# focegueda1998/CALM-ViT-DTE

Hardware: AMD Instinct MI355X
Metric: training images/sec (224^2, bs=256/GPU) (higher is better)
Workload: dtype f32; 1 GPU; CALM-ViT small224 cls, 224x224x3 synthetic, bs=256/GPU, fp32 matmuls, fwd+loss+bwd+clip+AdamW; batch resident in HBM when the timed region starts (the trainer's H2D copy of the batch is excluded); global_batch=256, parallelism=dp1, world=1, backend=none (single process), hipgraph=False

## Files before the change

calm-vit-dte_amd/_lib.py:

```python
import ctypes as C
import os

HERE = os.path.dirname(os.path.abspath(__file__))
LIB_PATH = os.environ.get("CALM_VIT_LIB") or os.path.join(HERE, "libcalmvit_hip.so")

ACT_NONE, ACT_GELU, ACT_GELU_BWD = 0, 1, 2
F32 = 0
ST_F32, ST_BF16, ST_FP8_E4M3, ST_FP8_E5M2 = 0, 1, 2, 3
E_INVAL, E_LAYOUT, E_UNSUPP = -1, -2, -3
ABI_VERSION = 7

_p = C.c_void_p
_i32 = C.c_int32
_i64 = C.c_int64
_f32 = C.c_float


class GemmArgs(C.Structure):
    _fields_ = [
        ("A", _p), ("B", _p), ("C", _p),
        ("M", _i32), ("N", _i32), ("K", _i32),
        ("batch0", _i32), ("batch1", _i32),
        ("a_rs", _i64), ("a_cs", _i64), ("a_b0", _i64), ("a_b1", _i64),
        ("b_rs", _i64), ("b_cs", _i64), ("b_b0", _i64), ("b_b1", _i64),
# ... 78 lines not shown
    "calm_gemm": (_i32, [C.POINTER(GemmArgs), _p]),
    "calm_gemm_workspace_bytes": (_i64, [C.POINTER(GemmArgs)]),
    "calm_gemm_set_option": (C.c_int, [_i32, _i32]),
    "calm_gemm_describe": (_i32, [C.POINTER(GemmArgs), C.POINTER(GemmPlan)]),
    "calm_reduce_scratch_floats": (_i64, [_i32, _i64, _i32]),
    "calm_layernorm_fwd": (_i32, [_p, _p, _p, _p, _p, _i64, _i32, _f32, _i32, _p]),
    "calm_layernorm_bwd": (_i32, [_p, _p, _p, _p, _p, _p, _p, _p, _i64, _i32, _i32, _p, _p]),
    "calm_cast_chunk_elems": (_i32, []),
    "calm_cast_bf16": (_i32, [_p, _p, _i32, _p]),
    "calm_cast_bf16_one": (_i32, [_p, _p, _i64, _p]),
    "calm_cast_f32_one": (_i32, [_p, _p, _i64, _p]),
    "calm_quantize_fp8": (_i32, [_p, _i32, _i64, _p, _i32, _p, _p]),
    "calm_transpose_u8": (_i32, [_p, _p, _i32, _i32, _p]),
    "calm_rope_fwd": (_i32, [_p, _p, _p, _p, _p, _i32, _i32, _i32, _i32, _i32, _i32, _i32, _i32, _p]),
    "calm_rope_bwd": (_i32, [_p, _p, _p, _p, _p, _p, _i32, _i32, _i32, _i32, _i32, _i32, _i32, _i32, _i32, _p, _p]),
    "calm_softmax_fwd": (_i32, [_p, _i64, _i32, _p]),
    "calm_softmax_bwd": (_i32, [_p, _p, _i64, _i32, _p]),
    "calm_softmax_bwd_heads": (_i32, [_p, _p, _p, _i32, _i32, _i32, _i32, _p]),
    "calm_sum_heads": (_i32, [_p, _p, _i32, _i32, _i64, _p]),
    "calm_attention_fwd_supported": (_i32, [_i32, _i32, _i32, _i32]),
    "calm_attention_fwd": (_i32, [_p] * 15 + [_i32] * 5 + [_p]),
    "calm_attention_bwd_preferred": (_i32, [_i32, _i32, _i32, _i32]),
    "calm_attention_bwd": (_i32, [_p] * 10 + [_i32] * 5 + [_p]),
    "calm_attention_fwd_lse": (_i32, [_p] * 15 + [_i32] * 5 + [_p]),
    "calm_attention_bwd_lse_scratch_bytes": (_i64, [_i32] * 5),
    "calm_attention_bwd_lse": (_i32, [_p] * 7 + [_i64] + [_p] * 4 + [_i32] * 5 + [_p]),
    "calm_attention_infer": (_i32, [_p] * 11 + [_i32] * 5 + [_p]),
    "calm_attention16_supported": (_i32, [_i32, _i32, _i32]),
    "calm_attention16_fwd": (_i32, [_p] * 16 + [_i32] * 4 + [_p]),
    "calm_attention16_bwd": (_i32, [_p] * 13 + [_i32] * 4 + [_p]),
    "calm_attention16_infer": (_i32, [_p] * 11 + [_i32] * 4 + [_p]),
    "calm_latent_fwd": (_i32, [_p, _p, _p, _p, _p, _i64, _i32, _p, _p]),
    "calm_latent_bwd": (_i32, [_p, _p, _p, _p, _p, _p, _i64, _i32, _p]),
    "calm_sn_plan": (_i32, [C.POINTER(SnLayer), _i32, _p, C.POINTER(SnPlanInfo)]),
    "calm_sn_power_iter": (_i32, [_p, C.POINTER(SnPlanInfo), _i32, _f32, _p, _p]),
    "calm_sn_weight_bwd": (_i32, [_p, _p, _p, _p, _p, _p, _p, _p, _i32, _i32, _p, _p]),
    "calm_optim_chunk_elems": (_i32, []),
    "calm_optim_step": (_i32, [_p, _i32, _p, _i32, _p, C.POINTER(OptimHparams), _p, _p, _p, _p, _p]),
    "calm_ema_chunk_elems": (_i32, []),
    "calm_ema_update": (_i32, [_p, _i32, _p, _i32, _f32, _i32, _p, _p, _p, _p]),
    "calm_ema_swap": (_i32, [_p, _i32, _p, _i32, _p]),
    "calm_collate_mix": (_i32, [_p, _p, _p, _i32, _i32, _i32, _i32, _f32, _p, _p, _p, _p]),
    "calm_collate_crop_mix": (_i32, [_p, _i32, _i32, _p, _p, _p, _i32, _i32, _i32, _i32, _i32, _f32, _p, _p, _p, _p]),
    "calm_augment_collate": (_i32, [_p, _i32, _i32, _p, _p, _p, _i32, _i32, _i32, _i32, _i32, _f32, _p, _p, _p, _p]),
    "calm_resize_coeffs": (_i32, [_i32, _i32, _p, _p, _i32]),
    "calm_resize_u8": (_i32, [_p, _i64, _p, _p, _i32, _i32, _i32, _p]),
# ... 51 lines not shown
```

calm-vit-dte_amd/backend.py:

```python
import contextlib
import ctypes as C
import os

import numpy as np
import torch

from . import _lib
from ._lib import ACT_GELU, ACT_GELU_BWD, ACT_NONE

SN_EPS = 1e-12

GEMM_WORKSPACE = os.environ.get("CALM_GEMM_WORKSPACE", "1") != "0"
BF16_STORAGE = os.environ.get("CALM_BF16_STORAGE", "1") != "0"
PRECISIONS = {"fp32": 0, "bf16": 1, "bf16x3": 2, "fp8": 1}
FP8_DTYPES = (torch.float8_e4m3fn, torch.float8_e5m2)
_precision = "fp32"


def set_matmul_precision(name):
    global _precision
    if name not in PRECISIONS:
        raise ValueError(f"unknown matmul precision {name!r}; choose from {sorted(PRECISIONS)}")
    _precision = name

# ... 1 lines not shown
def get_matmul_precision():
    return _precision


ATTENTION_STORAGES = ("probs", "lse")


def _check_attention_storage(name):
    if name not in ATTENTION_STORAGES:
        raise ValueError(f"unknown attention storage {name!r}; choose from {sorted(ATTENTION_STORAGES)}")
    return name


_attention_storage = _check_attention_storage(os.environ.get("CALM_ATTN_STORAGE") or "probs")


def set_attention_storage(name):
    global _attention_storage
    _attention_storage = _check_attention_storage(name)


def get_attention_storage():
    return _attention_storage


_lean_inference = os.environ.get("CALM_LEAN_INFERENCE", "0") not in ("", "0")


def set_lean_inference(on):
    global _lean_inference
    _lean_inference = bool(on)


def get_lean_inference():
    return _lean_inference


def lean_forward():
    return _lean_inference and not torch.is_grad_enabled()


_loss_kernels = os.environ.get("CALM_LOSS_KERNELS", "0") not in ("", "0")


def set_loss_kernels(on):
    global _loss_kernels
# ... 541 lines not shown
    def softmax_bwd_heads(self, p, dp, dm, B, H, Sq, cols):
        _lib.check(self.lib.calm_softmax_bwd_heads(_ptr(p), _ptr(dp), _ptr(dm), B, H, Sq, cols, _stream()),
                   "calm_softmax_bwd_heads")

    def sum_heads(self, dl, dm, B, H, per_head):
        _lib.check(self.lib.calm_sum_heads(_ptr(dl), _ptr(dm), B, H, per_head, _stream()), "calm_sum_heads")

    def attn_fwd_supported(self, Sq, Skv, H, hd):
        return bool(self.lib.calm_attention_fwd_supported(Sq, Skv, H, hd))

    def attn_fwd(self, q, k, v, w1, b1, s1, w2, b2, s2, out, R, hp, hg, Mk, P, B, Sq, Skv, H, hd):
        _lib.check(self.lib.calm_attention_fwd(_ptr(q), _ptr(k), _ptr(v), _ptr(w1), _ptr(b1), _ptr(s1), _ptr(w2),
                                               _ptr(b2), _ptr(s2), _ptr(out), _ptr(R), _ptr(hp), _ptr(hg),
                                               _ptr(Mk), _ptr(P, True), B, Sq, Skv, H, hd, _stream()), "calm_attention_fwd")

    def attn_bwd_preferred(self, Sq, Skv, H, hd):
        return bool(self.lib.calm_attention_bwd_preferred(Sq, Skv, H, hd))

    def attn_bwd(self, q, k, v, dout, P, dS, dq, dk, dv, dM, B, Sq, Skv, H, hd):
        _lib.check(self.lib.calm_attention_bwd(_ptr(q), _ptr(k), _ptr(v), _ptr(dout), _ptr(P), _ptr(dS), _ptr(dq),
                                               _ptr(dk), _ptr(dv), _ptr(dM), B, Sq, Skv, H, hd, _stream()),
                   "calm_attention_bwd")

    def attn_fwd_lse(self, q, k, v, w1, b1, s1, w2, b2, s2, out, R, hp, hg, Mk, lse, B, Sq, Skv, H, hd):
        _lib.check(self.lib.calm_attention_fwd_lse(_ptr(q), _ptr(k), _ptr(v), _ptr(w1), _ptr(b1), _ptr(s1), _ptr(w2),
                                                   _ptr(b2), _ptr(s2), _ptr(out), _ptr(R), _ptr(hp), _ptr(hg),
                                                   _ptr(Mk), _ptr(lse), B, Sq, Skv, H, hd, _stream()),
                   "calm_attention_fwd_lse")

    def attn_bwd_lse_scratch_bytes(self, B, Sq, Skv, H, hd):
        return int(self.lib.calm_attention_bwd_lse_scratch_bytes(B, Sq, Skv, H, hd))

    def attn_bwd_lse(self, q, k, v, dout, Mk, lse, scratch, dq, dk, dv, dM, B, Sq, Skv, H, hd):
        if scratch is None or not scratch.is_cuda or not scratch.is_contiguous():
            raise TypeError("attn_bwd_lse: contiguous CUDA scratch tensor expected")
        _lib.check(self.lib.calm_attention_bwd_lse(_ptr(q), _ptr(k), _ptr(v), _ptr(dout), _ptr(Mk), _ptr(lse),
                                                   scratch.data_ptr(), scratch.numel() * scratch.element_size(),
                                                   _ptr(dq), _ptr(dk), _ptr(dv), _ptr(dM), B, Sq, Skv, H, hd, _stream()),
                   "calm_attention_bwd_lse")

    def attn_infer(self, q, k, v, w1, b1, s1, w2, b2, s2, out, Mk, B, Sq, Skv, H, hd):
        _lib.check(self.lib.calm_attention_infer(_ptr(q), _ptr(k), _ptr(v), _ptr(w1), _ptr(b1), _ptr(s1), _ptr(w2),
                                                 _ptr(b2), _ptr(s2), _ptr(out), _ptr(Mk), B, Sq, Skv, H, hd, _stream()),
                   "calm_attention_infer")

    def attn16_supported(self, S, H, hd):
# ... 164 lines not shown
```

calm-vit-dte_amd/csrc/attention_fused.hip:

```cpp
#include "common.h"

#ifndef ATT_TR_ROWFAST
#define ATT_TR_ROWFAST 1
#endif

namespace {

typedef float f32x4v __attribute__((ext_vector_type(4)));

struct AttnFwdP {
    const float* q; const float* k; const float* v;
    const float* w1; const float* b1; const float* s1;
    const float* w2; const float* b2; const float* s2;
    float* out;
    float* R; float* hp; float* hg; float* Mk; float* P;
    int B, Sq, Skv, H, hd;
    float scale;
    float* lse;
};

constexpr int NV_Q = 1;

template <int NV> struct Regs { f32x4v v[NV]; };

// ... 73 lines not shown
    static constexpr int SKV = 16 * NJ, TQ = 16 * NW;
    static constexpr int LDJ = ld_km(SKV), LDQ = ld_km(TQ);
    static constexpr int LDN1 = 20;
    static constexpr int LDJ2 = SKV + 4;
    static_assert(LDJ % 32 == 16 && LDQ % 32 == 16, "K-major strides: lane groups 16 banks apart");
    static constexpr int Q_OFF = 32 * LDJ, V_OFF = Q_OFF + 32 * LDQ;
    __device__ static float* buf_k(float* smem, int i) { return smem + i * 16 * LDJ; }
    __device__ static float* buf_q(float* smem, int i) { return smem + Q_OFF + i * 16 * LDQ; }
    static constexpr int W2_OFF = 2 * SKV * LDN1, PH2 = W2_OFF + 32 * LDJ2;
    __device__ static float* buf_w1(float* smem, int i) { return smem + i * SKV * LDN1; }
    __device__ static float* buf_w2(float* smem, int i) { return smem + W2_OFF + i * 16 * LDJ2; }
    struct Hd { int DT, hdp, LDV, stripe; };
    __host__ __device__ static constexpr Hd at(int hd) {
        const int DT = (hd + 15) / 16;
        const int hdp = 16 * DT, LDV = hdp + 4;
        return {DT, hdp, LDV, SKV * LDV};
    }
    static constexpr size_t fwd_bytes(int hd) {
        const int ph13 = V_OFF + at(hd).stripe;
        return sizeof(float) * (size_t)(ph13 > PH2 ? ph13 : PH2);
    }
    static constexpr size_t bwd_q_bytes(int hd) { return sizeof(float) * (size_t)(V_OFF + at(hd).stripe); }
    static constexpr size_t bwd_kv_bytes(int hd) { return sizeof(float) * (size_t)at(hd).stripe; }
};

template <int NJ, int NW, bool LEAN>
__global__ __launch_bounds__(64 * NW) void attn_fwd_kernel(const AttnFwdP p) {
    constexpr int NTH = 64 * NW;
    constexpr int NV_K = (NJ + NW - 1) / NW;
    extern __shared__ __attribute__((aligned(16))) float smem[];
    typedef AttGeo<NJ, NW> G;
    constexpr int SKV = G::SKV, LDJ = G::LDJ, LDN1 = G::LDN1, LDJ2 = G::LDJ2;

    const int tid = threadIdx.x, lane = tid & 63, wave = tid >> 6;
    constexpr int TQ = G::TQ, LDQ = G::LDQ;
    const int r16 = lane & 15, g = lane >> 4;
    const int b = blockIdx.y;
    const int q0 = blockIdx.x * TQ;
    const int nq = min(TQ, p.Sq - q0);
    const bool active = 16 * wave < nq;
    const int iq = q0 + 16 * wave + r16;
    const int D = p.H * p.hd;

    const float* qb = p.q + ((long)b * p.Sq + q0) * D;
    const float* kb = p.k + (long)b * p.Skv * D;
    const float* vb = p.v + (long)b * p.Skv * D;
// ... 238 lines not shown
                    for (int r = 0; r < 4; ++r) {
                        accO = MFMA16(vcol[(16 * t + 4 * g + r) * LDV], accS[t][r], accO);
                        accO2 = MFMA16(vcol[(16 * t + 4 * g + r) * LDV + d2], accS[t][r], accO2);
                    }
                if (16 * d + 4 * g < hd) *reinterpret_cast<f32x4v*>(orow + 16 * d + 4 * g) = accO;
                if (d + 1 < DT && 16 * (d + 1) + 4 * g < hd)
                    *reinterpret_cast<f32x4v*>(orow + 16 * (d + 1) + 4 * g) = accO2;
            }
        }
        __syncthreads();
    }
}

struct AttnBwdP {
    const float* q; const float* k; const float* v; const float* dout;
    const float* P;
    float* dS;
    float* dq; float* dk; float* dv;
    float* dM;
    int B, Sq, Skv, H, hd;
    float scale;
    const float* Mk;
    const float* lse;
};

template <int NJ, int NW, bool LSE>
__global__ __launch_bounds__(64 * NW) void attn_bwd_q_kernel(const AttnBwdP p) {
    constexpr int NTH = 64 * NW;
    constexpr int NV_K = (NJ + NW - 1) / NW;
    extern __shared__ __attribute__((aligned(16))) float smem[];
    typedef AttGeo<NJ, NW> G;
    constexpr int SKV = G::SKV, LDJ = G::LDJ, TQ = G::TQ, LDQ = G::LDQ;
    const int tid = threadIdx.x, lane = tid & 63, wave = tid >> 6;
    const int r16 = lane & 15, g = lane >> 4;
    const int b = blockIdx.y;
    const int q0 = blockIdx.x * TQ;
    const int nq = min(TQ, p.Sq - q0);
    const bool active = 16 * wave < nq;
    const int iq = q0 + 16 * wave + r16;
    const int D = p.H * p.hd;
    const int hd = p.hd;
    const auto gh = G::at(hd);
    const int DT = gh.DT, hdp = gh.hdp, LDV = gh.LDV;
    auto bufK = [&](int i) { return G::buf_k(smem, i); };
    auto bufQ = [&](int i) { return G::buf_q(smem, i); };
    float* bufV = smem + G::V_OFF;
// ... 174 lines not shown
                const float* kcol = bufV + 16 * d + r16;
                const int d2 = (d + 1 < DT) ? 16 : 0;
#pragma unroll
                for (int t = 0; t < NJ; ++t)
#pragma unroll
                    for (int r = 0; r < 4; ++r) {
                        accO = MFMA16(kcol[(16 * t + 4 * g + r) * LDV], accD[t][r], accO);
                        accO2 = MFMA16(kcol[(16 * t + 4 * g + r) * LDV + d2], accD[t][r], accO2);
                    }
                if (16 * d + 4 * g < hd) *reinterpret_cast<f32x4v*>(qrow + 16 * d + 4 * g) = accO * p.scale;
                if (d + 1 < DT && 16 * (d + 1) + 4 * g < hd)
                    *reinterpret_cast<f32x4v*>(qrow + 16 * (d + 1) + 4 * g) = accO2 * p.scale;
            }
        }
        __syncthreads();
    }
    if (active) {
        float* mrow = p.dM + ((long)b * p.Sq + iq) * p.Skv;
#pragma unroll
        for (int t = 0; t < NJ; ++t) *reinterpret_cast<f32x4v*>(mrow + 16 * t + 4 * g) = accM[t];
    }
}

template <int NI, int NW>
__global__ __launch_bounds__(64 * NW) void attn_bwd_kv_kernel(const AttnBwdP p) {
    constexpr int NTH = 64 * NW;
    extern __shared__ __attribute__((aligned(16))) float smem[];
    typedef AttGeo<NI, NW> G;
    constexpr int SQ = G::SKV, TK = G::TQ;
    const int tid = threadIdx.x, lane = tid & 63, wave = tid >> 6;
    const int r16 = lane & 15, g = lane >> 4;
    const int b = blockIdx.y;
    const int k0 = blockIdx.x * TK;
    const int nk = min(TK, p.Skv - k0);
    const bool active = 16 * wave < nk;
    const int jk = k0 + 16 * wave + r16;
    const int D = p.H * p.hd;
    const int hd = p.hd;
    const auto gh = G::at(hd);
    const int DT = gh.DT, hdp = gh.hdp, LDV = gh.LDV;
    float* bufV = smem;
    const int v_per_row = hdp >> 2, v_total = SQ * v_per_row;
    const float* qb = p.q + (long)b * p.Sq * D;
    const float* dob = p.dout + (long)b * p.Sq * D;

    constexpr int SB = 4;
    auto stage = [&](const float* src) {
#pragma unroll 1
        for (int f0 = tid; f0 < v_total; f0 += SB * NTH) {
            f32x4v val[SB];
#pragma unroll
            for (int u = 0; u < SB; ++u) {
                const int f = f0 + u * NTH;
                const int row = f / v_per_row, cq = f - row * v_per_row;
                val[u] = (f32x4v){0.f, 0.f, 0.f, 0.f};
                if (f < v_total && 4 * cq < hd) val[u] = *reinterpret_cast<const f32x4v*>(src + (long)row * D + 4 * cq);
            }
#pragma unroll
            for (int u = 0; u < SB; ++u) {
                const int f = f0 + u * NTH;
                const int row = f / v_per_row, cq = f - row * v_per_row;
                if (f < v_total) *reinterpret_cast<f32x4v*>(bufV + row * LDV + 4 * cq) = val[u];
            }
        }
    };
    auto contract = [&](const f32x4v (&X)[NI], float* out_row, float scale) {
#pragma unroll 1
        for (int d = 0; d < DT; d += 2) {
            f32x4v accO = {0.f, 0.f, 0.f, 0.f}, accO2 = {0.f, 0.f, 0.f, 0.f};
            const float* col = bufV + 16 * d + r16;
            const int d2 = (d + 1 < DT) ? 16 : 0;
#pragma unroll
            for (int t = 0; t < NI; ++t)
#pragma unroll
                for (int r = 0; r < 4; ++r) {
                    accO = MFMA16(col[(16 * t + 4 * g + r) * LDV], X[t][r], accO);
                    accO2 = MFMA16(col[(16 * t + 4 * g + r) * LDV + d2], X[t][r], accO2);
                }
            if (16 * d + 4 * g < hd) *reinterpret_cast<f32x4v*>(out_row + 16 * d + 4 * g) = accO * scale;
            if (d + 1 < DT && 16 * (d + 1) + 4 * g < hd)
                *reinterpret_cast<f32x4v*>(out_row + 16 * (d + 1) + 4 * g) = accO2 * scale;
        }
    };

#pragma unroll 1
    for (int h = 0; h < p.H; ++h) {
        const long base = ((long)b * p.H + h) * p.Sq * p.Skv + (active ? jk : k0);
        f32x4v X[NI];
#pragma unroll
        for (int t = 0; t < NI; ++t)
#pragma unroll
            for (int r = 0; r < 4; ++r) X[t][r] = p.P[base + (long)(16 * t + 4 * g + r) * p.Skv];
        stage(dob + h * hd);
        __syncthreads();
        if (active) contract(X, p.dv + ((long)b * p.Skv + jk) * D + h * hd, 1.0f);
        __syncthreads();
#pragma unroll
        for (int t = 0; t < NI; ++t)
#pragma unroll
            for (int r = 0; r < 4; ++r) X[t][r] = p.dS[base + (long)(16 * t + 4 * g + r) * p.Skv];
        stage(qb + h * hd);
        __syncthreads();
        if (active) contract(X, p.dk + ((long)b * p.Skv + jk) * D + h * hd, p.scale);
        __syncthreads();
    }
}

template <class P>
int launch(void (*kernel)(const P), dim3 grid, int threads, size_t lds, hipStream_t s, const P& p) {
    hipError_t e = hipFuncSetAttribute(reinterpret_cast<const void*>(kernel), hipFuncAttributeMaxDynamicSharedMemorySize,
                                       (int)lds);
    if (e != hipSuccess) return (int)e;
    hipLaunchKernelGGL(kernel, grid, dim3(threads), lds, s, p);
    CALM_LAUNCH_CHECK();
    return 0;
}

template <class G, bool LSE>
int launch_bwd(const AttnBwdP& p, hipStream_t s) {
    static_assert(G::fwd_bytes(4) <= LDS_MAX, "fits at the smallest head dim; larger ones are checked per launch");
    constexpr int NJ = G::NJ, NW = G::NW;
    const int tiles = p.Sq / 16;
    dim3 grid((tiles + NW - 1) / NW, p.B);
    const int e = launch(&attn_bwd_q_kernel<NJ, NW, LSE>, grid, 64 * NW, G::bwd_q_bytes(p.hd), s, p);
    if (e) return e;
    return launch(&attn_bwd_kv_kernel<NJ, NW>, grid, 64 * NW, G::bwd_kv_bytes(p.hd), s, p);
}

template <class G, bool LEAN>
int launch_fwd(const AttnFwdP& p, hipStream_t s) {
    static_assert(G::fwd_bytes(4) <= LDS_MAX, "fits at the smallest head dim; larger ones are checked per launch");
    constexpr int NJ = G::NJ, NW = G::NW;
    const int tiles = p.Sq / 16;
    const size_t lds = G::fwd_bytes(p.hd);
    if (lds > LDS_MAX) return CALM_E_UNSUPP;
    dim3 grid((tiles + NW - 1) / NW, p.B);
    return launch(&attn_fwd_kernel<NJ, NW, LEAN>, grid, 64 * NW, lds, s, p);
}

#ifndef ATT_NW11
#define ATT_NW11 11
#endif
#ifndef ATT_NW14
#define ATT_NW14 7
#endif

template <class F>
int with_geo(int nj, F&& f) {
    switch (nj) {
        case 2: return f(AttGeo<2, 2>{});
        case 3: return f(AttGeo<3, 3>{});
        case 5: return f(AttGeo<5, 5>{});
        case 8: return f(AttGeo<8, 8>{});
        case 11: return f(AttGeo<11, ATT_NW11>{});
        case 14: return f(AttGeo<14, ATT_NW14>{});
    }
    return CALM_E_UNSUPP;
}

int attention_bwd_dispatch(const AttnBwdP& p, bool lse, hipStream_t s) {
    return with_geo(p.Skv / 16, [&](auto g) -> int {
        typedef decltype(g) G;
        return lse ? launch_bwd<G, true>(p, s) : launch_bwd<G, false>(p, s);
    });
}

}

extern "C" {

int calm_attention_fwd_supported(int32_t Sq, int32_t Skv, int32_t H, int32_t hd) {
    if (Sq <= 0 || Skv <= 0 || H <= 0 || hd <= 0) return 0;
    if (Sq != Skv || (Sq & 15) || (hd & 3) || hd > 128) return 0;
    return with_geo(Skv / 16, [&](auto g) -> int { return decltype(g)::fwd_bytes(hd) <= LDS_MAX ? 1 : 0; }) == 1;
}

namespace {
int attention_fwd(const float* q, const float* k, const float* v, const float* w1, const float* b1, const float* s1,
                  const float* w2, const float* b2, const float* s2, float* out, float* R, float* hp, float* hg, float* Mk,
                  float* P, float* lse, int32_t B, int32_t Sq, int32_t Skv, int32_t H, int32_t hd, void* stream) {
    if (!q || !k || !v || !w1 || !b1 || !s1 || !w2 || !b2 || !s2 || !out || !R || !hp || !hg || !Mk || B <= 0)
        return CALM_E_INVAL;
    if (!calm_attention_fwd_supported(Sq, Skv, H, hd)) return CALM_E_UNSUPP;
    if (B > 65535) return CALM_E_UNSUPP;
    AttnFwdP p{q, k, v, w1, b1, s1, w2, b2, s2, out, R, hp, hg, Mk, P, B, Sq, Skv, H, hd, 1.0f / sqrtf((float)hd), lse};
    hipStream_t s = as_stream(stream);
// ... 18 lines not shown

int calm_attention_infer(const float* q, const float* k, const float* v, const float* w1, const float* b1,
                         const float* s1, const float* w2, const float* b2, const float* s2, float* out, float* Mk,
                         int32_t B, int32_t Sq, int32_t Skv, int32_t H, int32_t hd, void* stream) {
    if (!q || !k || !v || !w1 || !b1 || !s1 || !w2 || !b2 || !s2 || !out || !Mk || B <= 0) return CALM_E_INVAL;
    if (!calm_attention_fwd_supported(Sq, Skv, H, hd)) return CALM_E_UNSUPP;
    if (B > 65535) return CALM_E_UNSUPP;
    AttnFwdP p{q, k, v, w1, b1, s1, w2, b2, s2, out, nullptr, nullptr, nullptr, Mk, nullptr, B, Sq, Skv, H, hd,
               1.0f / sqrtf((float)hd), nullptr};
    hipStream_t s = as_stream(stream);
    return with_geo(Skv / 16, [&](auto g) -> int { return launch_fwd<decltype(g), true>(p, s); });
}

int calm_attention_bwd_preferred(int32_t Sq, int32_t Skv, int32_t H, int32_t hd) {
    return calm_attention_fwd_supported(Sq, Skv, H, hd) && (hd <= 64 || Skv / 16 == 11);
}

int calm_attention_bwd(const float* q, const float* k, const float* v, const float* dout, const float* P, float* dS,
                       float* dq, float* dk, float* dv, float* dM, int32_t B, int32_t Sq, int32_t Skv, int32_t H,
                       int32_t hd, void* stream) {
    if (!q || !k || !v || !dout || !P || !dS || !dq || !dk || !dv || !dM || B <= 0) return CALM_E_INVAL;
    if (!calm_attention_fwd_supported(Sq, Skv, H, hd)) return CALM_E_UNSUPP;
    if (B > 65535) return CALM_E_UNSUPP;
    AttnBwdP p{q, k, v, dout, P, dS, dq, dk, dv, dM, B, Sq, Skv, H, hd, 1.0f / sqrtf((float)hd), nullptr, nullptr};
    return attention_bwd_dispatch(p, false, as_stream(stream));
}

int64_t calm_attention_bwd_lse_scratch_bytes(int32_t B, int32_t Sq, int32_t Skv, int32_t H, int32_t hd) {
    if (B <= 0 || B > 65535 || !calm_attention_fwd_supported(Sq, Skv, H, hd)) return 0;
    return 2 * (int64_t)sizeof(float) * B * H * Sq * Skv;
}

int calm_attention_bwd_lse(const float* q, const float* k, const float* v, const float* dout, const float* Mk,
                           const float* lse, void* scratch, int64_t scratch_bytes, float* dq, float* dk, float* dv,
                           float* dM, int32_t B, int32_t Sq, int32_t Skv, int32_t H, int32_t hd, void* stream) {
    if (!q || !k || !v || !dout || !Mk || !lse || !scratch || !dq || !dk || !dv || !dM || B <= 0) return CALM_E_INVAL;
    const int64_t need = calm_attention_bwd_lse_scratch_bytes(B, Sq, Skv, H, hd);
    if (need == 0) return CALM_E_UNSUPP;
    if (scratch_bytes < need || (reinterpret_cast<uintptr_t>(scratch) & 15)) return CALM_E_INVAL;
    float* P = static_cast<float*>(scratch);
    float* dS = P + need / (2 * (int64_t)sizeof(float));
    AttnBwdP p{q, k, v, dout, P, dS, dq, dk, dv, dM, B, Sq, Skv, H, hd, 1.0f / sqrtf((float)hd), Mk, lse};
    return attention_bwd_dispatch(p, true, as_stream(stream));
}

}
```

calm-vit-dte_amd/ops.py:

```python
import math
import os
import threading

import torch
from torch.autograd import Function
from torch.autograd.function import once_differentiable

from .backend import (ACT_GELU, ACT_GELU_BWD, ACT_NONE, act_dtype, bf16_pipeline, effective_precision, fp8_linears,
                      get_attention_storage, get_backend)
from .spectral_norm import W16_ATTR, W16_GEN_ATTR

_amp_fwd = torch.amp.custom_fwd(device_type="cuda")
_amp_bwd = torch.amp.custom_bwd(device_type="cuda")

GROUP_PROJECTIONS = os.environ.get("CALM_GROUP_PROJECTIONS", "1") != "0"
FUSE_LN_SKIP = os.environ.get("CALM_FUSE_LN_SKIP", "1") != "0"

_noise_override = None


def set_noise_override(fn):
    global _noise_override
    _noise_override = fn


def draw_noise(like):
    return _noise_override(like) if _noise_override is not None else torch.randn_like(like)


_dropout_key_override = None


# ... 489 lines not shown
        table = torch.empty(2 * S * (dr // 2), dtype=torch.float32, device=xr.device)
        out = torch.empty(B, S, H * (dc + dr), dtype=torch.bfloat16 if out16 else torch.float32, device=xr.device)
        be.rope_fwd(content, xr, inv_freq, table, out, B, S, H, dc, dr)
        ctx.dims = (B, S, H, dc, dr)
        ctx.content_dtype = content.dtype if content is not None else None
        ctx.save_for_backward(xr, table)
        return out

    @staticmethod
    @once_differentiable
    @_amp_bwd
    def backward(ctx, dout):
        be = get_backend()
        xr, table = ctx.saved_tensors
        B, S, H, dc, dr = ctx.dims
        dout = _c(dout)
        d_xr = torch.empty_like(xr)
        d_content = torch.empty(B, S, H * dc, dtype=ctx.content_dtype, device=xr.device) if dc > 0 else None
        d_if = _zeros((dr // 2,), table)
        be.rope_bwd(dout, xr, table, d_content, d_xr, d_if, B, S, H, dc, dr)
        return d_content, d_xr, d_if, None, None


def _attn_mask_bwd(be, defer, dM, q, k, dq, dk, R, hp, hg, w1, w2, u1, v1, s1, u2, v2, s2, w1o=None, w2o=None):
    w1o, w2o = w1 if w1o is None else w1o, w2 if w2o is None else w2o
    B, Sq, D = q.shape
    Skv = k.shape[1]
    dev, dt = q.device, q.dtype
    G2 = _zeros_big(w2.shape, w2)
    _lin_wgrad(be, dM, hg, G2)
    dW2, _ = _sn_wbwd(be, G2, w2, u2, v2, s2, defer=defer[1])
    db2 = _colsum(be, dM)
    dhp = torch.empty_like(hp)
    _lin_dgrad(be, dM, w2o, s2, dhp, act=ACT_GELU_BWD, aux=hp)
    R2 = R.view(B * Sq, Skv)
    G1 = _zeros_big(w1.shape, w1)
    _lin_wgrad(be, dhp, R2, G1)
    dW1, _ = _sn_wbwd(be, G1, w1, u1, v1, s1, defer=defer[0])
    db1 = _colsum(be, dhp)
    dR = torch.empty(B, Sq, Skv, dtype=dt, device=dev)
    _lin_dgrad(be, dhp, w1o, s1, dR.view(B * Sq, Skv))
    be.gemm(dR, k, dq, Sq, D, Skv, (Skv, 1, Sq * Skv, 0), (1, D, Skv * D, 0), (D, Sq * D, 0), batch=(B, 1),
            accumulate=True)
    be.gemm(dR, q, dk, Skv, D, Sq, (1, Skv, Sq * Skv, 0), (1, D, Sq * D, 0), (D, Skv * D, 0), batch=(B, 1),
            accumulate=True)
    return dW1, db1, dW2, db2


class LatentMaskAttentionFn(Function):

    @staticmethod
    @_amp_fwd
    def forward(ctx, q, k, v, w1, b1, w2, b2, u1, v1, s1, u2, v2, s2, H):
        be = get_backend()
        q, k, v = _c(q), _c(k), _c(v)
        B, Sq, D = q.shape
        Skv = k.shape[1]
        hd = D // H
        dev, dt = q.device, q.dtype
        R = torch.empty(B, Sq, Skv, dtype=dt, device=dev)
        hp = torch.empty(B * Sq, w1.shape[0], dtype=dt, device=dev)
        hg = torch.empty_like(hp)
        P = torch.empty(B, H, Sq, Skv, dtype=dt, device=dev)
        out = torch.empty(B, Sq, D, dtype=dt, device=dev)
        if be.attn_fwd_supported(Sq, Skv, H, hd):
            Mk = torch.empty(B * Sq, Skv, dtype=dt, device=dev)
# ... 12 lines not shown
                    batch=(B, H))
        ctx.H = H
        ctx.defer = (_deferred(w1), _deferred(w2))
        ctx.save_for_backward(q, k, v, R, hp, hg, P, w1, w2, u1, v1, s1, u2, v2, s2)
        return out

    @staticmethod
    @once_differentiable
    @_amp_bwd
    def backward(ctx, dout):
        be = get_backend()
        q, k, v, R, hp, hg, P, w1, w2, u1, v1, s1, u2, v2, s2 = ctx.saved_tensors
        H = ctx.H
        B, Sq, D = q.shape
        Skv = k.shape[1]
        hd = D // H
        scale = 1.0 / math.sqrt(hd)
        dout = _c(dout)
        dev, dt = q.device, q.dtype
        pb = (H * Sq * Skv, Sq * Skv)
        dP = torch.empty_like(P)
        dv, dq, dk = torch.empty_like(v), torch.empty_like(q), torch.empty_like(k)
        dM = torch.empty(B * Sq, Skv, dtype=dt, device=dev)
        if be.attn_bwd_preferred(Sq, Skv, H, hd):
            be.attn_bwd(q, k, v, dout, P, dP, dq, dk, dv, dM, B, Sq, Skv, H, hd)
        else:
            be.gemm(dout, v, dP, Sq, Skv, hd, (D, 1, Sq * D, hd), (D, 1, Skv * D, hd), (Skv,) + pb, batch=(B, H))
            be.gemm(P, dout, dv, Skv, hd, Sq, (1, Skv) + pb, (1, D, Sq * D, hd), (D, Skv * D, hd), batch=(B, H))
            be.softmax_bwd_heads(P, dP, dM, B, H, Sq, Skv)
            be.gemm(dP, k, dq, Sq, hd, Skv, (Skv, 1) + pb, (1, D, Skv * D, hd), (D, Sq * D, hd), batch=(B, H),
                    alpha=scale)
            be.gemm(dP, q, dk, Skv, hd, Sq, (1, Skv) + pb, (1, D, Sq * D, hd), (D, Skv * D, hd), batch=(B, H),
                    alpha=scale)
        dW1, db1, dW2, db2 = _attn_mask_bwd(be, ctx.defer, dM, q, k, dq, dk, R, hp, hg, w1, w2, u1, v1, s1, u2, v2, s2)
        return dq, dk, dv, dW1, db1, dW2, db2, None, None, None, None, None, None, None


class LatentMaskAttentionLseFn(Function):

    @staticmethod
    @_amp_fwd
    def forward(ctx, q, k, v, w1, b1, w2, b2, u1, v1, s1, u2, v2, s2, H):
        be = get_backend()
        q, k, v = _c(q), _c(k), _c(v)
        B, Sq, D = q.shape
        Skv = k.shape[1]
        hd = D // H
# ... 456 lines not shown
```

calm-vit-dte_amd/trainer.py:

```python
import contextlib
import os
import weakref

import torch
import torch.distributed as dist


def init_distributed(use_gpu=True):
    if int(os.environ.get("WORLD_SIZE", "1")) <= 1:
        return 0, 0, 1
    rank, world = int(os.environ["RANK"]), int(os.environ["WORLD_SIZE"])
    local_rank = int(os.environ.get("LOCAL_RANK", rank))
    os.environ.setdefault("HSA_ENABLE_IPC_MODE_LEGACY", "0")
    if not dist.is_initialized():
        backend = os.environ.get("CALM_DIST_BACKEND", "nccl" if use_gpu else "gloo")
        if use_gpu and backend == "nccl":
            torch.cuda.set_device(local_rank)
            dist.init_process_group(backend="nccl", device_id=torch.device("cuda", local_rank))
        elif use_gpu:
            torch.cuda.set_device(int(os.environ.get("CALM_LOCAL_DEVICE", local_rank)))
            dist.init_process_group(backend=backend)
        else:
            dist.init_process_group(backend="gloo")
    return rank, local_rank, world
# ... 1022 lines not shown
                               metrics=metrics, ema=ema)
        self.opt = optimizer
        if isinstance(optimizer, FusedClipAdamW):
            optimizer.lr_on_device = True
        self.x = example_x.clone()
        self.y = example_y.clone()
        snap = None
        if restore_after_warmup:
            if not isinstance(optimizer, FusedClipAdamW):
                raise ValueError("restore_after_warmup needs FusedClipAdamW (its whole state is a known set of tensors)")
            live = list(model.parameters()) + list(model.buffers()) + optimizer.exp_avg + optimizer.exp_avg_sq + \
                [optimizer._plan.step_dev] + ([metrics.buf] if metrics is not None else []) + \
                ([] if ema is None else ema.state_tensors())
            snap = ([(t, t.detach().clone()) for t in live], torch.cuda.get_rng_state(example_x.device),
                    None if scaler is None or not scaler.is_enabled() else scaler.get_scale())
        side = torch.cuda.Stream()
        side.wait_stream(torch.cuda.current_stream())
        with torch.cuda.stream(side):
            for _ in range(max(warmup, 1 if scaler is not None else 0)):
                self.inner(self.x, self.y)
        torch.cuda.current_stream().wait_stream(side)
        torch.cuda.synchronize()
        self.graph = torch.cuda.CUDAGraph()
        with torch.cuda.graph(self.graph):
            self.loss, self.y_hat = self.inner(self.x, self.y)
        if snap is not None:
            with torch.no_grad():
                for t, c in snap[0]:
                    t.copy_(c)
            torch.cuda.set_rng_state(snap[1], example_x.device)
            if snap[2] is not None:
                scaler.update(new_scale=float(snap[2]))
                if hasattr(self.inner, "_clean_steps"):
                    self.inner._clean_steps.zero_()
            torch.cuda.synchronize()

    def __call__(self, x, y_soft):
        self.x.copy_(x, non_blocking=True)
        self.y.copy_(y_soft, non_blocking=True)
        if isinstance(self.opt, FusedClipAdamW):
            self.opt.sync_lr_to_device()
        self.graph.replay()
        return self.loss, self.y_hat


class SoftMixCollate:

# ... 207 lines not shown
```

include/calm_vit.h:

```cpp
#ifndef CALM_VIT_H
#define CALM_VIT_H

#include <stddef.h>
#include <stdint.h>

#ifdef __cplusplus
extern "C" {
#endif

#define CALM_ABI_VERSION 7

#define CALM_E_INVAL   (-1)
#define CALM_E_LAYOUT  (-2)
#define CALM_E_UNSUPP  (-3)

enum { CALM_F32 = 0, CALM_BF16 = 1, CALM_BF16X3 = 2 };
enum { CALM_ST_F32 = 0, CALM_ST_BF16 = 1, CALM_ST_FP8_E4M3 = 2, CALM_ST_FP8_E5M2 = 3 };
enum { CALM_ACT_NONE = 0, CALM_ACT_GELU = 1, CALM_ACT_GELU_BWD = 2 };

int         calm_abi_version(void);
const char* calm_build_info(void);

typedef struct calm_gemm_args {
    const void* A; const void* B; void* C;
// ... 64 lines not shown
int calm_rope_bwd(const void* d_out, const void* xr, const float* table,
                  void* d_content, void* d_xr, float* d_inv_freq,
                  int32_t B, int32_t S, int32_t H, int32_t dc, int32_t dr,
                  int32_t dout_type, int32_t xr_type, int32_t dcontent_type, int32_t dxr_type,
                  float* partials , void* stream);

int calm_softmax_fwd(float* x, int64_t rows, int32_t cols, void* stream);
int calm_softmax_bwd(const float* p, float* dp, int64_t rows, int32_t cols, void* stream);
int calm_softmax_bwd_heads(const float* p, float* dp, float* dm, int32_t B, int32_t H, int32_t Sq, int32_t cols,
                           void* stream);
int calm_sum_heads(const float* dl, float* dm, int32_t B, int32_t H, int64_t per_head, void* stream);

int calm_attention_fwd_supported(int32_t Sq, int32_t Skv, int32_t H, int32_t hd);
int calm_attention_fwd(const float* q, const float* k, const float* v, const float* w1, const float* b1,
                       const float* s1, const float* w2, const float* b2, const float* s2, float* out, float* R,
                       float* hp, float* hg, float* Mk, float* P, int32_t B, int32_t Sq, int32_t Skv, int32_t H, int32_t hd,
                       void* stream);

int calm_attention_bwd_preferred(int32_t Sq, int32_t Skv, int32_t H, int32_t hd);
int calm_attention_bwd(const float* q, const float* k, const float* v, const float* dout, const float* P, float* dS,
                       float* dq, float* dk, float* dv, float* dM, int32_t B, int32_t Sq, int32_t Skv, int32_t H,
                       int32_t hd, void* stream);

int calm_attention_fwd_lse(const float* q, const float* k, const float* v, const float* w1, const float* b1,
                           const float* s1, const float* w2, const float* b2, const float* s2, float* out, float* R,
                           float* hp, float* hg, float* Mk, float* lse, int32_t B, int32_t Sq, int32_t Skv, int32_t H,
                           int32_t hd, void* stream);
int64_t calm_attention_bwd_lse_scratch_bytes(int32_t B, int32_t Sq, int32_t Skv, int32_t H, int32_t hd);
int calm_attention_bwd_lse(const float* q, const float* k, const float* v, const float* dout, const float* Mk,
                           const float* lse, void* scratch, int64_t scratch_bytes, float* dq, float* dk, float* dv,
                           float* dM, int32_t B, int32_t Sq, int32_t Skv, int32_t H, int32_t hd, void* stream);

int calm_attention_infer(const float* q, const float* k, const float* v, const float* w1, const float* b1,
                         const float* s1, const float* w2, const float* b2, const float* s2, float* out, float* Mk,
                         int32_t B, int32_t Sq, int32_t Skv, int32_t H, int32_t hd, void* stream);

int calm_attention16_supported(int32_t S, int32_t H, int32_t hd);
int calm_attention16_fwd(const void* q, const void* k, const void* v, const void* w1, const float* b1, const float* s1,
                         const void* w2, const float* b2, const float* s2, void* out, void* R, void* hp, void* hg,
                         void* Mk, void* MkT, float* lse, int32_t B, int32_t S, int32_t H, int32_t hd, void* stream);
int calm_attention16_bwd(const void* q, const void* k, const void* v, const void* out, const void* dout, const void* Mk,
                         const void* MkT, const float* lse, float* delta, void* dq, void* dk, void* dv, void* dM,
                         int32_t B, int32_t S, int32_t H, int32_t hd, void* stream);
int calm_attention16_infer(const void* q, const void* k, const void* v, const void* w1, const float* b1, const float* s1,
                           const void* w2, const float* b2, const float* s2, void* out, void* Mk, int32_t B, int32_t S,
                           int32_t H, int32_t hd, void* stream);
// ... 177 lines not shown
```

Before: 1933 images/sec.

## Add software-pipelined attention dK/dV backward kernel with optional dR fold

Adds a new attention backward kernel for dK/dV that double-buffers the staged dout/q stripes in LDS and prefetches the next head's P/dS tiles and rows into registers with buffer loads while the current contraction runs. It is enabled by default through the dispatch. The older kv kernel is also switched to buffer-resource loads with read-ahead in the contraction. An opt-in mode splits the backward into q and kv launches so the mask-gradient dR@q term can be folded into the dK contraction instead of a separate batched GEMM. The pipelined kernel costs more LDS and registers and forces a waves-per-EU occupancy setting.

```diff
diff --git a/calm-vit-dte_amd/_lib.py b/calm-vit-dte_amd/_lib.py
--- a/calm-vit-dte_amd/_lib.py
+++ b/calm-vit-dte_amd/_lib.py
@@ -124,6 +124,8 @@
     "calm_attention_fwd": (_i32, [_p] * 15 + [_i32] * 5 + [_p]),
     "calm_attention_bwd_preferred": (_i32, [_i32, _i32, _i32, _i32]),
     "calm_attention_bwd": (_i32, [_p] * 10 + [_i32] * 5 + [_p]),
+    "calm_attention_bwd_q": (_i32, [_p] * 8 + [_i32] * 5 + [_p]),
+    "calm_attention_bwd_kv": (_i32, [_p] * 7 + [_i32] * 5 + [_p]),
     "calm_attention_fwd_lse": (_i32, [_p] * 15 + [_i32] * 5 + [_p]),
     "calm_attention_bwd_lse_scratch_bytes": (_i64, [_i32] * 5),
     "calm_attention_bwd_lse": (_i32, [_p] * 7 + [_i64] + [_p] * 4 + [_i32] * 5 + [_p]),
diff --git a/calm-vit-dte_amd/backend.py b/calm-vit-dte_amd/backend.py
--- a/calm-vit-dte_amd/backend.py
+++ b/calm-vit-dte_amd/backend.py
@@ -47,6 +47,18 @@
 
 def get_attention_storage():
     return _attention_storage
+
+
+_attention_dr_fold = os.environ.get("CALM_ATTN_DR_FOLD", "0") not in ("", "0")
+
+
+def set_attention_dr_fold(on):
+    global _attention_dr_fold
+    _attention_dr_fold = bool(on)
+
+
+def get_attention_dr_fold():
+    return _attention_dr_fold
 
 
 _lean_inference = os.environ.get("CALM_LEAN_INFERENCE", "0") not in ("", "0")
@@ -634,6 +646,14 @@
                                                _ptr(dk), _ptr(dv), _ptr(dM), B, Sq, Skv, H, hd, _stream()),
                    "calm_attention_bwd")
 
+    def attn_bwd_q(self, q, k, v, dout, P, dS, dq, dM, B, Sq, Skv, H, hd):
+        _lib.check(self.lib.calm_attention_bwd_q(_ptr(q), _ptr(k), _ptr(v), _ptr(dout), _ptr(P), _ptr(dS), _ptr(dq),
+                                                 _ptr(dM), B, Sq, Skv, H, hd, _stream()), "calm_attention_bwd_q")
+
+    def attn_bwd_kv(self, q, dout, P, dS, dR, dk, dv, B, Sq, Skv, H, hd):
+        _lib.check(self.lib.calm_attention_bwd_kv(_ptr(q), _ptr(dout), _ptr(P), _ptr(dS), _ptr(dR, True), _ptr(dk),
+                                                  _ptr(dv), B, Sq, Skv, H, hd, _stream()), "calm_attention_bwd_kv")
+
     def attn_fwd_lse(self, q, k, v, w1, b1, s1, w2, b2, s2, out, R, hp, hg, Mk, lse, B, Sq, Skv, H, hd):
         _lib.check(self.lib.calm_attention_fwd_lse(_ptr(q), _ptr(k), _ptr(v), _ptr(w1), _ptr(b1), _ptr(s1), _ptr(w2),
                                                    _ptr(b2), _ptr(s2), _ptr(out), _ptr(R), _ptr(hp), _ptr(hg),
diff --git a/calm-vit-dte_amd/csrc/attention_fused.hip b/calm-vit-dte_amd/csrc/attention_fused.hip
--- a/calm-vit-dte_amd/csrc/attention_fused.hip
+++ b/calm-vit-dte_amd/csrc/attention_fused.hip
@@ -119,6 +119,16 @@
     }
     static constexpr size_t bwd_q_bytes(int hd) { return sizeof(float) * (size_t)(V_OFF + at(hd).stripe); }
     static constexpr size_t bwd_kv_bytes(int hd) { return sizeof(float) * (size_t)at(hd).stripe; }
+    static constexpr size_t bwd_kv2_bytes(int hd) { return 2 * bwd_kv_bytes(hd); }
+    static constexpr int kv2_ns(int hdp) { return (SKV * (hdp / 4) + 64 * NW - 1) / (64 * NW); }
+    static constexpr int kv2_hdp() {
+        int hdp = 0;
+        for (int h = 16; h <= 128; h += 16)
+            if (2 * sizeof(float) * (size_t)SKV * (h + 4) <= LDS_MAX && (NW <= 8 || kv2_ns(h) <= 6)) hdp = h;
+        return hdp;
+    }
+    static constexpr int KV2_HDP = kv2_hdp();
+    static constexpr int KV2_NS = kv2_ns(KV2_HDP);
 };
 
 template <int NJ, int NW, bool LEAN>
@@ -403,6 +413,7 @@
     float scale;
     const float* Mk;
     const float* lse;
+    const float* dR;
 };
 
 template <int NJ, int NW, bool LSE>
@@ -623,6 +634,66 @@
     }
 }
 
+__device__ __forceinline__ __amdgpu_buffer_rsrc_t kv_rsrc(const float* base, long bytes) {
+    const unsigned long long b = reinterpret_cast<unsigned long long>(base);
+    const unsigned lo = (unsigned)__builtin_amdgcn_readfirstlane((int)(unsigned)b);
+    const unsigned hi = (unsigned)__builtin_amdgcn_readfirstlane((int)(unsigned)(b >> 32));
+    return __builtin_amdgcn_make_buffer_rsrc(reinterpret_cast<void*>(((unsigned long long)hi << 32) | lo), 0, (int)bytes,
+                                             0x00020000);
+}
+template <int NI>
+__device__ __forceinline__ void kv_tiles(f32x4v (&X)[NI], __amdgpu_buffer_rsrc_t planes, unsigned voff, unsigned soff) {
+    constexpr int SKV = 16 * NI;
+#pragma unroll
+    for (int t = 0; t < NI; ++t)
+#pragma unroll
+        for (int r = 0; r < 4; ++r)
+            X[t][r] = __builtin_bit_cast(float, __builtin_amdgcn_raw_buffer_load_b32(
+                                                    planes, voff + 4 * r * SKV, soff + 4 * 16 * t * SKV, 0));
+}
+template <int NI>
+__device__ __forceinline__ void kv_fold(f32x4v (&X)[NI], const f32x4v (&dS)[NI], float scale) {
+#pragma unroll
+    for (int t = 0; t < NI; ++t)
+#pragma unroll
+        for (int r = 0; r < 4; ++r) X[t][r] = fmaf(scale, dS[t][r], X[t][r]);
+}
+template <bool AHEAD, int NI>
+__device__ __forceinline__ void kv_contract(const f32x4v (&X)[NI], const float* stripe, int LDV, int DT, int hd, int r16,
+                                            int g, float* out_row, float scale) {
+    constexpr int A = AHEAD ? 1 : 0;
+#pragma unroll 1
+    for (int d = 0; d < DT; d += 2) {
+        f32x4v accO = {0.f, 0.f, 0.f, 0.f}, accO2 = {0.f, 0.f, 0.f, 0.f};
+        const float* col = stripe + 16 * d + r16 + 4 * g * LDV;
+        const int d2 = (d + 1 < DT) ? 16 : 0;
+        float a[2][4], a2[2][4];
+        auto read = [&](int t) {
+#pragma unroll
+            for (int r = 0; r < 4; ++r) {
+                a[t & A][r] = col[(16 * t + r) * LDV];
+                a2[t & A][r] = col[(16 * t + r) * LDV + d2];
+            }
+        };
+        if (AHEAD) read(0);
+#pragma unroll
+        for (int t = 0; t < NI; ++t) {
+            if (!AHEAD) read(t);
+            else if (t + 1 < NI) read(t + 1);
+            __builtin_amdgcn_sched_barrier(0);
+#pragma unroll
+            for (int r = 0; r < 4; ++r) {
+                accO = MFMA16(a[t & A][r], X[t][r], accO);
+                accO2 = MFMA16(a2[t & A][r], X[t][r], accO2);
+            }
+            __builtin_amdgcn_sched_barrier(0);
+        }
+        if (16 * d + 4 * g < hd) *reinterpret_cast<f32x4v*>(out_row + 16 * d + 4 * g) = accO * scale;
+        if (d + 1 < DT && 16 * (d + 1) + 4 * g < hd)
+            *reinterpret_cast<f32x4v*>(out_row + 16 * (d + 1) + 4 * g) = accO2 * scale;
+    }
+}
+
 template <int NI, int NW>
 __global__ __launch_bounds__(64 * NW) void attn_bwd_kv_kernel(const AttnBwdP p) {
     constexpr int NTH = 64 * NW;
@@ -644,6 +715,12 @@
     const int v_per_row = hdp >> 2, v_total = SQ * v_per_row;
     const float* qb = p.q + (long)b * p.Sq * D;
     const float* dob = p.dout + (long)b * p.Sq * D;
+    const float fk = p.dR ? 1.0f : p.scale;
+    const unsigned voff = 4 * (4 * g * SQ + (active ? jk : k0));
+    const unsigned plane = 4 * SQ * SQ;
+    const auto Prs = kv_rsrc(p.P + (long)b * p.H * SQ * SQ, (long)p.H * plane);
+    const auto dSrs = kv_rsrc(p.dS + (long)b * p.H * SQ * SQ, (long)p.H * plane);
+    const auto dRrs = kv_rsrc(p.dR ? p.dR + (long)b * SQ * SQ : p.dS, plane);
 
     constexpr int SB = 4;
     auto stage = [&](const float* src) {
@@ -665,45 +742,114 @@
             }
         }
     };
-    auto contract = [&](const f32x4v (&X)[NI], float* out_row, float scale) {
-#pragma unroll 1
-        for (int d = 0; d < DT; d += 2) {
-            f32x4v accO = {0.f, 0.f, 0.f, 0.f}, accO2 = {0.f, 0.f, 0.f, 0.f};
-            const float* col = bufV + 16 * d + r16;
-            const int d2 = (d + 1 < DT) ? 16 : 0;
-#pragma unroll
-            for (int t = 0; t < NI; ++t)
-#pragma unroll
-                for (int r = 0; r < 4; ++r) {
-                    accO = MFMA16(col[(16 * t + 4 * g + r) * LDV], X[t][r], accO);
-                    accO2 = MFMA16(col[(16 * t + 4 * g + r) * LDV + d2], X[t][r], accO2);
-                }
-            if (16 * d + 4 * g < hd) *reinterpret_cast<f32x4v*>(out_row + 16 * d + 4 * g) = accO * scale;
-            if (d + 1 < DT && 16 * (d + 1) + 4 * g < hd)
-                *reinterpret_cast<f32x4v*>(out_row + 16 * (d + 1) + 4 * g) = accO2 * scale;
-        }
-    };
 
 #pragma unroll 1
     for (int h = 0; h < p.H; ++h) {
-        const long base = ((long)b * p.H + h) * p.Sq * p.Skv + (active ? jk : k0);
         f32x4v X[NI];
-#pragma unroll
-        for (int t = 0; t < NI; ++t)
-#pragma unroll
-            for (int r = 0; r < 4; ++r) X[t][r] = p.P[base + (long)(16 * t + 4 * g + r) * p.Skv];
+        kv_tiles(X, Prs, voff, h * plane);
         stage(dob + h * hd);
         __syncthreads();
-        if (active) contract(X, p.dv + ((long)b * p.Skv + jk) * D + h * hd, 1.0f);
+        if (active) kv_contract<true>(X, bufV, LDV, DT, hd, r16, g, p.dv + ((long)b * p.Skv + jk) * D + h * hd, 1.0f);
         __syncthreads();
-#pragma unroll
-        for (int t = 0; t < NI; ++t)
-#pragma unroll
-            for (int r = 0; r < 4; ++r) X[t][r] = p.dS[base + (long)(16 * t + 4 * g + r) * p.Skv];
+        if (p.dR) {
+            f32x4v dSt[NI];
+            kv_tiles(dSt, dSrs, voff, h * plane);
+            kv_tiles(X, dRrs, voff, 0);
+            kv_fold(X, dSt, p.scale);
+        } else {
+            kv_tiles(X, dSrs, voff, h * plane);
+        }
         stage(qb + h * hd);
         __syncthreads();
-        if (active) contract(X, p.dk + ((long)b * p.Skv + jk) * D + h * hd, p.scale);
+        if (active) kv_contract<true>(X, bufV, LDV, DT, hd, r16, g, p.dk + ((long)b * p.Skv + jk) * D + h * hd, fk);
         __syncthreads();
+    }
+}
+
+constexpr int kv2_waves(int NW) { return NW >= 7 ? (NW + 3) / 4 : NW == 5 ? 3 : 4; }
+
+template <int NI, int NW>
+__global__ __launch_bounds__(64 * NW) __attribute__((amdgpu_waves_per_eu(kv2_waves(NW), kv2_waves(NW))))
+void attn_bwd_kv2_kernel(const AttnBwdP p) {
+    constexpr int NTH = 64 * NW;
+    extern __shared__ __attribute__((aligned(16))) float smem[];
+    typedef AttGeo<NI, NW> G;
+    constexpr int SQ = G::SKV, TK = G::TQ, NS = G::KV2_NS;
+    const int tid = threadIdx.x, lane = tid & 63, wave = tid >> 6;
+    const int r16 = lane & 15, g = lane >> 4;
+    const int b = blockIdx.y;
+    const int k0 = blockIdx.x * TK;
+    const int nk = min(TK, p.Skv - k0);
+    const bool active = 16 * wave < nk;
+    const int jk = k0 + 16 * wave + r16;
+    const int D = p.H * p.hd;
+    const int hd = p.hd;
+    const auto gh = G::at(hd);
+    const int DT = gh.DT, hdp = gh.hdp, LDV = gh.LDV;
+    const int v_per_row = hdp >> 2, v_total = SQ * v_per_row;
+    const unsigned voff = 4 * (4 * g * SQ + (active ? jk : k0));
+    const unsigned plane = 4 * SQ * SQ;
+    const float* Pb = p.P + (long)b * p.H * SQ * SQ;
+    const float* dSb = p.dS + (long)b * p.H * SQ * SQ;
+    const float* qb = p.q + (long)b * SQ * D;
+    const float* dob = p.dout + (long)b * SQ * D;
+    const bool fold = p.dR != nullptr;
+    const auto dRrs = kv_rsrc(fold ? p.dR + (long)b * SQ * SQ : dSb, plane);
+    const unsigned orow = jk * D;
+    float* dvb = p.dv + (long)b * SQ * D;
+    float* dkb = p.dk + (long)b * SQ * D;
+    const float fk = fold ? 1.0f : p.scale;
+
+    Regs<NS> rs;
+    auto request = [&](const float* rows_b, int h) {
+        const auto rows = kv_rsrc(rows_b, 4l * SQ * D);
+#pragma unroll
+        for (int u = 0; u < NS; ++u) {
+            const int f = min(tid + u * NTH, v_total - 1);
+            const int row = f / v_per_row, cq = f - row * v_per_row;
+            rs.v[u] = __builtin_bit_cast(f32x4v, __builtin_amdgcn_raw_buffer_load_b128(
+                                                     rows, 4 * (row * D + min(4 * cq, hd - 4)), 4 * h * hd, 0));
+        }
+    };
+    auto commit = [&](float* dst) {
+#pragma unroll
+        for (int u = 0; u < NS; ++u) {
+            const int f = tid + u * NTH;
+            const int row = f / v_per_row, cq = f - row * v_per_row;
+            if (f < v_total) *reinterpret_cast<f32x4v*>(dst + row * LDV + 4 * cq) = rs.v[u];
+        }
+    };
+
+    f32x4v X[NI], Xn[NI];
+    auto zero = [&]() {
+#pragma unroll
+        for (int t = 0; t < NI; ++t) X[t] = (f32x4v){0.f, 0.f, 0.f, 0.f};
+    };
+    request(dob, 0);
+    kv_tiles(Xn, kv_rsrc(Pb, (long)p.H * plane), voff, 0);
+    zero();
+    commit(smem);
+    __syncthreads();
+    kv_fold(X, Xn, 1.0f);
+    const int nst = 2 * p.H;
+#pragma unroll 1
+    for (int n = 0; n < nst; ++n) {
+        const int h = n >> 1, hn = (n + 1) >> 1;
+        const bool ks = n & 1, more = n + 1 < nst;
+        if (more) {
+            request(ks ? dob : qb, hn);
+            kv_tiles(Xn, kv_rsrc(ks ? Pb : dSb, (long)p.H * plane), voff, hn * plane);
+        }
+        if (active)
+            kv_contract<(kv2_waves(NW) < 3)>(X, smem + (n & 1) * gh.stripe, LDV, DT, hd, r16, g,
+                                             (ks ? dkb : dvb) + h * hd + orow, ks ? fk : 1.0f);
+        if (more) {
+            const bool f = fold && !ks;
+            if (f) kv_tiles(X, dRrs, voff, 0); else zero();
+            commit(smem + ((n + 1) & 1) * gh.stripe);
+            __syncthreads();
+            kv_fold(X, Xn, f ? p.scale : 1.0f);
+        }
     }
 }
 
@@ -718,13 +864,23 @@
 }
 
 template <class G, bool LSE>
-int launch_bwd(const AttnBwdP& p, hipStream_t s) {
+int launch_bwd_q(const AttnBwdP& p, hipStream_t s) {
     static_assert(G::fwd_bytes(4) <= LDS_MAX, "fits at the smallest head dim; larger ones are checked per launch");
     constexpr int NJ = G::NJ, NW = G::NW;
     const int tiles = p.Sq / 16;
     dim3 grid((tiles + NW - 1) / NW, p.B);
-    const int e = launch(&attn_bwd_q_kernel<NJ, NW, LSE>, grid, 64 * NW, G::bwd_q_bytes(p.hd), s, p);
-    if (e) return e;
+    return launch(&attn_bwd_q_kernel<NJ, NW, LSE>, grid, 64 * NW, G::bwd_q_bytes(p.hd), s, p);
+}
+
+template <class G>
+int launch_bwd_kv(const AttnBwdP& p, hipStream_t s) {
+    static_assert(G::KV2_HDP >= 16 && G::bwd_kv2_bytes(G::KV2_HDP) <= LDS_MAX, "two stripes fit at the smallest head dim");
+    constexpr int NJ = G::NJ, NW = G::NW;
+    const int tiles = p.Sq / 16;
+    dim3 grid((tiles + NW - 1) / NW, p.B);
+    static const bool kv2 = [] { const char* e = getenv("CALM_ATTN_BWD_KV2"); return !(e && e[0] == '0'); }();
+    if (kv2 && G::at(p.hd).hdp <= G::KV2_HDP)
+        return launch(&attn_bwd_kv2_kernel<NJ, NW>, grid, 64 * NW, G::bwd_kv2_bytes(p.hd), s, p);
     return launch(&attn_bwd_kv_kernel<NJ, NW>, grid, 64 * NW, G::bwd_kv_bytes(p.hd), s, p);
 }
 
@@ -759,10 +915,16 @@
     return CALM_E_UNSUPP;
 }
 
-int attention_bwd_dispatch(const AttnBwdP& p, bool lse, hipStream_t s) {
+enum { BWD_Q = 1, BWD_KV = 2 };
+
+int attention_bwd_dispatch(const AttnBwdP& p, bool lse, int which, hipStream_t s) {
     return with_geo(p.Skv / 16, [&](auto g) -> int {
         typedef decltype(g) G;
-        return lse ? launch_bwd<G, true>(p, s) : launch_bwd<G, false>(p, s);
+        if (which & BWD_Q) {
+            const int e = lse ? launch_bwd_q<G, true>(p, s) : launch_bwd_q<G, false>(p, s);
+            if (e) return e;
+        }
+        return (which & BWD_KV) ? launch_bwd_kv<G>(p, s) : 0;
     });
 }
 
@@ -827,8 +989,28 @@
     if (!q || !k || !v || !dout || !P || !dS || !dq || !dk || !dv || !dM || B <= 0) return CALM_E_INVAL;
     if (!calm_attention_fwd_supported(Sq, Skv, H, hd)) return CALM_E_UNSUPP;
     if (B > 65535) return CALM_E_UNSUPP;
-    AttnBwdP p{q, k, v, dout, P, dS, dq, dk, dv, dM, B, Sq, Skv, H, hd, 1.0f / sqrtf((float)hd), nullptr, nullptr};
-    return attention_bwd_dispatch(p, false, as_stream(stream));
+    AttnBwdP p{q, k, v, dout, P, dS, dq, dk, dv, dM, B, Sq, Skv, H, hd, 1.0f / sqrtf((float)hd), nullptr, nullptr, nullptr};
+    return attention_bwd_dispatch(p, false, BWD_Q | BWD_KV, as_stream(stream));
+}
+
+int calm_attention_bwd_q(const float* q, const float* k, const float* v, const float* dout, const float* P, float* dS,
+                         float* dq, float* dM, int32_t B, int32_t Sq, int32_t Skv, int32_t H, int32_t hd, void* stream) {
+    if (!q || !k || !v || !dout || !P || !dS || !dq || !dM || B <= 0) return CALM_E_INVAL;
+    if (!calm_attention_fwd_supported(Sq, Skv, H, hd)) return CALM_E_UNSUPP;
+    if (B > 65535) return CALM_E_UNSUPP;
+    AttnBwdP p{q, k, v, dout, P, dS, dq, nullptr, nullptr, dM, B, Sq, Skv, H, hd, 1.0f / sqrtf((float)hd), nullptr, nullptr,
+               nullptr};
+    return attention_bwd_dispatch(p, false, BWD_Q, as_stream(stream));
+}
+
+int calm_attention_bwd_kv(const float* q, const float* dout, const float* P, const float* dS, const float* dR, float* dk,
+                          float* dv, int32_t B, int32_t Sq, int32_t Skv, int32_t H, int32_t hd, void* stream) {
+    if (!q || !dout || !P || !dS || !dk || !dv || B <= 0) return CALM_E_INVAL;
+    if (!calm_attention_fwd_supported(Sq, Skv, H, hd)) return CALM_E_UNSUPP;
+    if (B > 65535) return CALM_E_UNSUPP;
+    AttnBwdP p{q, nullptr, nullptr, dout, P, const_cast<float*>(dS), nullptr, dk, dv, nullptr, B, Sq, Skv, H, hd,
+               1.0f / sqrtf((float)hd), nullptr, nullptr, dR};
+    return attention_bwd_dispatch(p, false, BWD_KV, as_stream(stream));
 }
 
 int64_t calm_attention_bwd_lse_scratch_bytes(int32_t B, int32_t Sq, int32_t Skv, int32_t H, int32_t hd) {
@@ -845,8 +1027,8 @@
     if (scratch_bytes < need || (reinterpret_cast<uintptr_t>(scratch) & 15)) return CALM_E_INVAL;
     float* P = static_cast<float*>(scratch);
     float* dS = P + need / (2 * (int64_t)sizeof(float));
-    AttnBwdP p{q, k, v, dout, P, dS, dq, dk, dv, dM, B, Sq, Skv, H, hd, 1.0f / sqrtf((float)hd), Mk, lse};
-    return attention_bwd_dispatch(p, true, as_stream(stream));
-}
-
-}
+    AttnBwdP p{q, k, v, dout, P, dS, dq, dk, dv, dM, B, Sq, Skv, H, hd, 1.0f / sqrtf((float)hd), Mk, lse, nullptr};
+    return attention_bwd_dispatch(p, true, BWD_Q | BWD_KV, as_stream(stream));
+}
+
+}
diff --git a/calm-vit-dte_amd/ops.py b/calm-vit-dte_amd/ops.py
--- a/calm-vit-dte_amd/ops.py
+++ b/calm-vit-dte_amd/ops.py
@@ -7,7 +7,7 @@
 from torch.autograd.function import once_differentiable
 
 from .backend import (ACT_GELU, ACT_GELU_BWD, ACT_NONE, act_dtype, bf16_pipeline, effective_precision, fp8_linears,
-                      get_attention_storage, get_backend)
+                      get_attention_dr_fold, get_attention_storage, get_backend)
 from .spectral_norm import W16_ATTR, W16_GEN_ATTR
 
 _amp_fwd = torch.amp.custom_fwd(device_type="cuda")
@@ -543,7 +543,8 @@
         return d_content, d_xr, d_if, None, None
 
 
-def _attn_mask_bwd(be, defer, dM, q, k, dq, dk, R, hp, hg, w1, w2, u1, v1, s1, u2, v2, s2, w1o=None, w2o=None):
+def _attn_mask_bwd(be, defer, dM, q, k, dq, dk, R, hp, hg, w1, w2, u1, v1, s1, u2, v2, s2, w1o=None, w2o=None,
+                   fold_dk=False):
     w1o, w2o = w1 if w1o is None else w1o, w2 if w2o is None else w2o
     B, Sq, D = q.shape
     Skv = k.shape[1]
@@ -563,6 +564,8 @@
     _lin_dgrad(be, dhp, w1o, s1, dR.view(B * Sq, Skv))
     be.gemm(dR, k, dq, Sq, D, Skv, (Skv, 1, Sq * Skv, 0), (1, D, Skv * D, 0), (D, Sq * D, 0), batch=(B, 1),
             accumulate=True)
+    if fold_dk:
+        return dW1, db1, dW2, db2, dR
     be.gemm(dR, q, dk, Skv, D, Sq, (1, Skv, Sq * Skv, 0), (1, D, Sq * D, 0), (D, Skv * D, 0), batch=(B, 1),
             accumulate=True)
     return dW1, db1, dW2, db2
@@ -621,7 +624,14 @@
         dP = torch.empty_like(P)
         dv, dq, dk = torch.empty_like(v), torch.empty_like(q), torch.empty_like(k)
         dM = torch.empty(B * Sq, Skv, dtype=dt, device=dev)
-        if be.attn_bwd_preferred(Sq, Skv, H, hd):
+        fused = be.attn_bwd_preferred(Sq, Skv, H, hd)
+        if fused and get_attention_dr_fold() and getattr(be, "attn_bwd_kv", None) is not None:
+            be.attn_bwd_q(q, k, v, dout, P, dP, dq, dM, B, Sq, Skv, H, hd)
+            dW1, db1, dW2, db2, dR = _attn_mask_bwd(be, ctx.defer, dM, q, k, dq, dk, R, hp, hg, w1, w2, u1, v1, s1, u2,
+                                                    v2, s2, fold_dk=True)
+            be.attn_bwd_kv(q, dout, P, dP, dR, dk, dv, B, Sq, Skv, H, hd)
+            return dq, dk, dv, dW1, db1, dW2, db2, None, None, None, None, None, None, None
+        if fused:
             be.attn_bwd(q, k, v, dout, P, dP, dq, dk, dv, dM, B, Sq, Skv, H, hd)
         else:
             be.gemm(dout, v, dP, Sq, Skv, hd, (D, 1, Sq * D, hd), (D, 1, Skv * D, hd), (Skv,) + pb, batch=(B, H))
diff --git a/calm-vit-dte_amd/trainer.py b/calm-vit-dte_amd/trainer.py
--- a/calm-vit-dte_amd/trainer.py
+++ b/calm-vit-dte_amd/trainer.py
@@ -1068,7 +1068,8 @@
         torch.cuda.current_stream().wait_stream(side)
         torch.cuda.synchronize()
         self.graph = torch.cuda.CUDAGraph()
-        with torch.cuda.graph(self.graph):
+        mode = "thread_local" if reducer is not None else "global"
+        with torch.cuda.graph(self.graph, capture_error_mode=mode):
             self.loss, self.y_hat = self.inner(self.x, self.y)
         if snap is not None:
             with torch.no_grad():
diff --git a/include/calm_vit.h b/include/calm_vit.h
--- a/include/calm_vit.h
+++ b/include/calm_vit.h
@@ -110,6 +110,11 @@
                        float* dq, float* dk, float* dv, float* dM, int32_t B, int32_t Sq, int32_t Skv, int32_t H,
                        int32_t hd, void* stream);
 
+int calm_attention_bwd_q(const float* q, const float* k, const float* v, const float* dout, const float* P, float* dS,
+                         float* dq, float* dM, int32_t B, int32_t Sq, int32_t Skv, int32_t H, int32_t hd, void* stream);
+int calm_attention_bwd_kv(const float* q, const float* dout, const float* P, const float* dS, const float* dR, float* dk,
+                          float* dv, int32_t B, int32_t Sq, int32_t Skv, int32_t H, int32_t hd, void* stream);
+
 int calm_attention_fwd_lse(const float* q, const float* k, const float* v, const float* w1, const float* b1,
                            const float* s1, const float* w2, const float* b2, const float* s2, float* out, float* R,
                            float* hp, float* hg, float* Mk, float* lse, int32_t B, int32_t Sq, int32_t Skv, int32_t H,
```

Measured after the change: 1949 images/sec (median of 6 runs). Within noise of the previous version (+0.8%).
